# mhnazeri/PMoE

Hardware: AMD Instinct MI355X
Metric: samples/sec fwd+bwd, 256x256 RGB 4-expert PMoE (higher is better)
Workload: dtype bf16; 1 GPU; 4-expert MoE (PMoE experts), 256x256x3 x4 frames, batch 64/GPU, fwd+moe_loss+bwd, dropout 0.3; global_batch=64, parallelism=dp1

## Files before the change

pmoe_amd/csrc/conv_res.hip:

```cpp
#include "conv_common.h"
#include <stdlib.h>
#include "kernels.h"

template <int LOG_RB> __device__ __forceinline__ int rswz(int x) { return swz_chunk<LOG_RB, 0>(x); }

template <int LOG_RB, bool BIAS = false>
__global__ void __launch_bounds__(512) conv3x3_res_kernel(const ConvArgs a, const int tiles_per_expert,
                                                         const int wgs_per_expert, const int region_bytes) {
    constexpr int RB = 1 << LOG_RB, CPR = RB / 16, LOG_CPR = LOG_RB - 4;
    constexpr int KSUB = RB / 32;
    constexpr int VE = 8;
    constexpr int MAXV = 11;
    extern __shared__ __attribute__((aligned(16))) char smem[];

    const int tid = threadIdx.x, lane = tid & 63, wave = tid >> 6;
    const int grp = wave >> 2, gw = wave & 3, gtid = tid & 255;
    const int l31 = lane & 31, hh = lane >> 5;
    const int e = blockIdx.y, wg = blockIdx.x;
    const int t0 = (int)((long long)wg * tiles_per_expert / wgs_per_expert);
    const int t1 = (int)((long long)(wg + 1) * tiles_per_expert / wgs_per_expert);
    const int n = t1 - t0;

    const int lTW = a.lTW, lTH = a.lTH;
    const int TW = 1 << lTW, TH = 1 << lTH;
    const int PW = TW + 2, PH = TH + 2;
    const int NPIX = a.TN * PH * PW;

    char* Wl = smem;
    char* region = smem + 9 * 64 * RB + grp * region_bytes;

    float* lbias = reinterpret_cast<float*>(smem + 9 * 64 * RB + 2 * region_bytes);
    if (BIAS && tid < 64) lbias[tid] = a.bias[(size_t)e * a.CoutP + tid];
    {
        const bf16* wsrc = (const bf16*)a.w + (size_t)e * a.CoutP * 9 * a.Cin;
        for (int v = tid; v < 9 * 64 * CPR; v += 512) {
            const int j = v & (CPR - 1);
            const int row = (v >> LOG_CPR) & 63;
            const int tap = v >> (LOG_CPR + 6);
            const v4i val = ldg16(wsrc + ((size_t)row * 9 + tap) * a.Cin + j * VE);
            *reinterpret_cast<v4i*>(Wl + (tap * 64 + row) * RB + ((j ^ rswz<LOG_RB>(row)) << 4)) = val;
        }
    }

    auto geom = [&](int t, PatchGeom& g, int& n0, int& oy0, int& ox0) {
        int q = t0 + t;
        const int px = q % a.tiles_x; q /= a.tiles_x;
        const int py = q % a.tiles_y; q /= a.tiles_y;
        n0 = e * a.ipe + q * a.TN;
        oy0 = py * TH; ox0 = px * TW;
        g.n0 = n0; g.n_end = (e + 1) * a.ipe; g.e_first_img = e * a.ipe;
        g.Y0 = oy0 - 1; g.X0 = ox0 - 1; g.PH = PH; g.PW = PW; g.NPIX = NPIX;
        g.H = a.H; g.W = a.W; g.ld = a.in_ld; g.coff = a.in_coff; g.cmax = a.Cin;
        g.dilate = 0; g.shared = a.in_shared; g.step = 1;
    };

    const bf16* in = (const bf16*)a.in;
    PatchStage<bf16, LOG_RB, 256, MAXV> ps;
    auto issue_tile = [&](int t) {
        PatchGeom g; int n0, oy0, ox0;
        geom(t, g, n0, oy0, ox0);
        ps.issue(in, g, 0, gtid);
    };

    int ppb[2];
#pragma unroll
    for (int mt = 0; mt < 2; ++mt) {
        const int p = gw * 64 + mt * 32 + l31;
        const int mx = p & (TW - 1), my = (p >> lTW) & (TH - 1), pn = p >> (lTW + lTH);
        ppb[mt] = (pn * PH + my) * PW + mx;
    }
    int arow_off[2][KSUB];
#pragma unroll
    for (int nt = 0; nt < 2; ++nt)
#pragma unroll
        for (int ks = 0; ks < KSUB; ++ks) {
            const int row = nt * 32 + l31;
            arow_off[nt][ks] = row * RB + (((ks * 2 + hh) ^ rswz<LOG_RB>(row)) << 4);
        }

    f32x16 acc[2][2];
    float s1[VE], s2[VE];
#pragma unroll
    for (int i = 0; i < VE; ++i) s1[i] = s2[i] = 0.f;
    const int cc = gtid & 7, pr = gtid >> 3;
    const bool cvalid = cc * VE < a.Cout;
    bf16* out = (bf16*)a.out;
    const bf16* res = (const bf16*)a.res;

    if (grp == 0 && n > 0) {
        issue_tile(0);
        ps.template commit<0>(region, NPIX, gtid);
    }
    __syncthreads();

    auto taps = [&](int tap_lo) {
        int pb[2] = {ppb[0], ppb[1]};
        asm volatile("" : "+v"(pb[0]), "+v"(pb[1]));
#pragma unroll
        for (int tp = 0; tp < 3; ++tp) {
            const int tap = tap_lo + tp;
            const int tapoff = (tap / 3) * PW + (tap % 3);
            const char* wt = Wl + tap * 64 * RB;
            int pp[2], fp[2];
#pragma unroll
            for (int mt = 0; mt < 2; ++mt) {
                pp[mt] = pb[mt] + tapoff;
                fp[mt] = rswz<LOG_RB>(pp[mt]);
            }
#pragma unroll
            for (int ks = 0; ks < KSUB; ++ks) {
                v4i af[2], bfr[2];
#pragma unroll
                for (int nt = 0; nt < 2; ++nt) af[nt] = *reinterpret_cast<const v4i*>(wt + arow_off[nt][ks]);
#pragma unroll
                for (int mt = 0; mt < 2; ++mt)
                    bfr[mt] = *reinterpret_cast<const v4i*>(region + (pp[mt] << LOG_RB) + (((ks * 2 + hh) ^ fp[mt]) << 4));
#pragma unroll
                for (int nt = 0; nt < 2; ++nt)
#pragma unroll
                    for (int mt = 0; mt < 2; ++mt)
                        acc[nt][mt] = __builtin_amdgcn_mfma_f32_32x32x16_bf16(__builtin_bit_cast(bf16x8, af[nt]),
                                                                              __builtin_bit_cast(bf16x8, bfr[mt]),
                                                                              acc[nt][mt], 0, 0, 0);
            }
        }
    };

    for (int h = 0; h <= n; ++h) {
        if (grp == (h & 1)) {
            const bool live = h < n;
            if (live) {
                if (BIAS) {
#pragma unroll
                    for (int i = 0; i < 2; ++i)
#pragma unroll
                        for (int g = 0; g < 4; ++g) {
                            const f32x4 b = *reinterpret_cast<const f32x4*>(lbias + (i * 4 + g) * 8 + hh * 4);
#pragma unroll
                            for (int j = 0; j < 2; ++j)
#pragma unroll
                                for (int k = 0; k < 4; ++k) acc[i][j][4 * g + k] = b[k];
                        }
                } else {
#pragma unroll
                    for (int i = 0; i < 2; ++i)
#pragma unroll
                        for (int j = 0; j < 2; ++j)
#pragma unroll
                            for (int k = 0; k < 16; ++k) acc[i][j][k] = 0.f;
                }
                taps(0);
            }
            __syncthreads();
            if (live) taps(3);
            __syncthreads();
            if (live) taps(6);
            __syncthreads();
        } else {
            const bool have = h >= 1, next = h + 1 < n;
            PatchGeom gg; int n0 = 0, oy0 = 0, ox0 = 0;
            v4i rb[8];
            if (next) issue_tile(h + 1);
            if (have) {
                geom(h - 1, gg, n0, oy0, ox0);
#pragma unroll
                for (int nt = 0; nt < 2; ++nt)
#pragma unroll
                    for (int mt = 0; mt < 2; ++mt) {
                        const int p = gw * 64 + mt * 32 + l31;
#pragma unroll
                        for (int g = 0; g < 4; ++g) {
                            bf16x4 v;
#pragma unroll
                            for (int i = 0; i < 4; ++i) v[i] = (bf16)acc[nt][mt][4 * g + i];
                            *reinterpret_cast<bf16x4*>(region + p * 128 + (((nt * 4 + g) ^ (p & 7)) << 4) + 8 * hh) = v;
                        }
                    }
            }
            __syncthreads();
            if (have) {
#pragma unroll
                for (int u = 0; u < 8; ++u) {
                    const int p = pr + 32 * u;
                    rb[u] = *reinterpret_cast<const v4i*>(region + p * 128 + ((cc ^ (p & 7)) << 4));
                }
            }
            __syncthreads();
            if (next) ps.template commit<0>(region, NPIX, gtid);
            if (have) {
#pragma unroll
                for (int u = 0; u < 8; ++u) {
                    const int p = pr + 32 * u;
                    const int mx = p & (TW - 1), my = (p >> lTW) & (TH - 1), pn = p >> (lTW + lTH);
                    const int nn = n0 + pn, oy = oy0 + my, ox = ox0 + mx;
                    if (cvalid && nn < gg.n_end && oy < a.Ho && ox < a.Wo) {
                        const size_t opix = ((size_t)nn * a.Ho + oy) * a.Wo + ox;
                        v4i pk = rb[u];
                        if (a.res_mode == PMOE_RES_ADD) {
                            float v[VE], rv[VE];
                            unpack16<bf16>(rb[u], v);
                            unpack16<bf16>(ldg16(res + opix * a.res_ld + a.res_coff + cc * VE), rv);
#pragma unroll
                            for (int i = 0; i < VE; ++i) v[i] += rv[i];
                            pk = pack16<bf16>(v);
                        }
                        if (a.stats) {
                            float rr[VE];
                            unpack16<bf16>(pk, rr);
#pragma unroll
                            for (int i = 0; i < VE; ++i) { s1[i] += rr[i]; s2[i] += rr[i] * rr[i]; }
                        }
                        stg16(out + opix * a.out_ld + a.out_coff + cc * VE, pk);
                    }
                }
            }
            __syncthreads();
        }
    }

    if (a.stats) {
        __syncthreads();
        float* red = reinterpret_cast<float*>(smem);
#pragma unroll
        for (int i = 0; i < VE; ++i) {
#pragma unroll
            for (int off = 8; off < 64; off <<= 1) {
                s1[i] += __shfl_xor(s1[i], off);
                s2[i] += __shfl_xor(s2[i], off);
            }
        }
        if (lane < 8) {
#pragma unroll
            for (int i = 0; i < VE; ++i) {
                red[(wave * 2 + 0) * 64 + cc * VE + i] = s1[i];
                red[(wave * 2 + 1) * 64 + cc * VE + i] = s2[i];
            }
        }
        __syncthreads();
        if (tid < 128) {
            const int which = tid >> 6, c = tid & 63;
            float s = 0.f;
#pragma unroll
            for (int w = 0; w < 8; ++w) s += red[(w * 2 + which) * 64 + c];
            a.stats[(((size_t)e * wgs_per_expert + wg) * 2 + which) * a.CoutP + c] = s;
        }
    }
}

#ifdef PMOE_STAMP
#define RSTAMP_INIT unsigned long long st_prev = __builtin_amdgcn_s_memtime(); const unsigned long long st_r0 = __builtin_amdgcn_s_memrealtime(); unsigned st_acc[5] = {0, 0, 0, 0, 0};
#define RLAP(i) { const unsigned long long st_t = __builtin_amdgcn_s_memtime(); st_acc[i] += (unsigned)(st_t - st_prev); st_prev = st_t; }
#else
#define RSTAMP_INIT
#define RLAP(i)
#endif

template <bool BIAS>
__global__ void __launch_bounds__(512, 2) conv3x3_resdma_kernel(const ConvArgs a, const int tiles_per_expert,
                                                                const int wgs_per_expert, const int pbuf_bytes,
                                                                const int magic_pw, const int magic_ph) {
    constexpr int RB = 128, LOG_RBK = 7, VE = 8;
    typedef __attribute__((address_space(3))) void lds_void;
    extern __shared__ __attribute__((aligned(16))) char smem[];
    const int tid = threadIdx.x, lane = tid & 63;
    const int wave = __builtin_amdgcn_readfirstlane(tid >> 6);
    const int l31 = lane & 31, hh = lane >> 5;
    const int wm = wave >> 1, wn = wave & 1;
    const int e = blockIdx.y, wg = blockIdx.x;
    const int t0 = (int)((long long)wg * tiles_per_expert / wgs_per_expert);
    const int t1 = (int)((long long)(wg + 1) * tiles_per_expert / wgs_per_expert);
    const int ntile = t1 - t0;

    const int lTW = a.lTW, lTH = a.lTH;
    const int TW = 1 << lTW, TH = 1 << lTH;
    const int PW = TW + 2, PH = TH + 2;
    const int NPIX = a.TN * PH * PW;
    const int NPIECE = (NPIX + 7) >> 3;
    const int my_pieces = (NPIECE - wave + 7) >> 3;

    char* Wl = smem;
    char* pbuf = smem + 9 * 64 * RB;
    float* lbias = reinterpret_cast<float*>(pbuf + 2 * pbuf_bytes);
    if (BIAS && tid < 64) lbias[tid] = a.bias[(size_t)e * a.CoutP + tid];
    const bool dbn = a.res_mode == PMOE_RES_DBN;
    float* lbn = lbias + 64;
    if (dbn && tid < 256) {
        const int nset = a.N / a.bn_ipe;
        lbn[tid] = (tid & 63) < a.Cout ? a.bn[((size_t)(tid >> 6) * nset + (e * a.ipe) / a.bn_ipe) * a.Cout + (tid & 63)] : 0.f;
    }

    const bf16* inb = (const bf16*)a.in + (size_t)e * a.ipe * a.H * a.W * a.in_ld + a.in_coff;
    const __amdgpu_buffer_rsrc_t rs_in = __builtin_amdgcn_make_buffer_rsrc(
        (void*)inb, (short)0, (int)(((long long)a.ipe * a.H * a.W * a.in_ld - a.in_coff) * 2), 0x00020000);
    const bf16* wsrc = (const bf16*)a.w + (size_t)e * a.CoutP * 9 * a.Cin;
    const __amdgpu_buffer_rsrc_t rs_w = __builtin_amdgcn_make_buffer_rsrc((void*)wsrc, (short)0, 64 * 9 * 64 * 2, 0x00020000);
    constexpr int OOB = 0x7ff80000;

#pragma unroll
    for (int i = 0; i < 9; ++i) {
        const int piece = wave + 8 * i;
        const int tap = piece >> 3, row = ((piece & 7) << 3) + (lane >> 3);
        const int voff = ((row * 9 + tap) * 64 * 2) + (((lane & 7) ^ ((row >> 1) & 7)) << 4);
        __builtin_amdgcn_raw_ptr_buffer_load_lds(rs_w, (lds_void*)(Wl + (piece << 10)), 16, voff, 0, 0, 0);
    }

    auto tile_geo = [&](int t, int& n0, int& oy0, int& ox0) {
        int qq = t0 + t;
        const int px = qq % a.tiles_x; qq /= a.tiles_x;
        const int py = qq % a.tiles_y; qq /= a.tiles_y;
        n0 = qq * a.TN;
        oy0 = py * TH; ox0 = px * TW;
    };
    auto issue_patch = [&](int t, int buf) {
        int n0, oy0, ox0;
        tile_geo(t, n0, oy0, ox0);
#pragma unroll
        for (int i = 0; i < 6; ++i) {
            if (i < my_pieces) {
                const int pp = ((wave + 8 * i) << 3) + (lane >> 3);
                const int rowq = (pp * magic_pw) >> 16, px = pp - rowq * PW;
                const int pn = (rowq * magic_ph) >> 16, prow = rowq - pn * PH;
                const int n = n0 + pn, Y = oy0 - 1 + prow, X = ox0 - 1 + px;
                const bool ok = pp < NPIX && n < a.ipe && (unsigned)Y < (unsigned)a.H && (unsigned)X < (unsigned)a.W;
                const int voff = ok ? ((((n * a.H + Y) * a.W + X) * a.in_ld) << 1) + (((lane & 7) ^ ((px >> 1) & 7)) << 4) : OOB;
                __builtin_amdgcn_raw_ptr_buffer_load_lds(rs_in, (lds_void*)(pbuf + buf * pbuf_bytes + ((wave + 8 * i) << 10)), 16,
                                                         voff, 0, 0, 0);
            }
        }
    };

    int pbase[2], pcol[2];
#pragma unroll
    for (int mt = 0; mt < 2; ++mt) {
        const int p = wm * 64 + mt * 32 + l31;
        const int mx = p & (TW - 1), my = (p >> lTW) & (TH - 1), pn = p >> (lTW + lTH);
        pbase[mt] = ((pn * PH + my) * PW + mx) << LOG_RBK;
        pcol[mt] = mx;
    }
    int aoff[4];
#pragma unroll
    for (int ks = 0; ks < 4; ++ks) {
        const int row = wn * 32 + l31;
        aoff[ks] = row * RB + (((ks * 2 + hh) ^ ((row >> 1) & 7)) << 4);
    }

    float s1[VE], s2[VE];
#pragma unroll
    for (int i = 0; i < VE; ++i) s1[i] = s2[i] = 0.f;
    const int cc = tid & 7, pr = tid >> 3;
    const bool cvalid = cc * VE < a.Cout;
    bf16* out = (bf16*)a.out;
    const bf16* res = (const bf16*)a.res;
    const bool res_pref = (a.res_mode == PMOE_RES_ADD || dbn) && a.prefetch;

    if (ntile > 0) issue_patch(0, 0);
    asm volatile("s_waitcnt vmcnt(0) lgkmcnt(0)" ::: "memory");
    __builtin_amdgcn_s_barrier();
    float kmu[VE], kis[VE], ksc[VE], ksh[VE];
#pragma unroll
    for (int i = 0; i < VE; ++i) kmu[i] = kis[i] = ksc[i] = ksh[i] = 0.f;
    if (dbn) {
#pragma unroll
        for (int i = 0; i < VE; ++i) {
            kmu[i] = lbn[cc * VE + i]; kis[i] = lbn[64 + cc * VE + i]; ksc[i] = lbn[128 + cc * VE + i]; ksh[i] = lbn[192 + cc * VE + i];
        }
    }

    RSTAMP_INIT
    for (int t = 0; t < ntile; ++t) {
        const int buf = t & 1;
        if (t + 1 < ntile) issue_patch(t + 1, buf ^ 1);
        v4i rpre[4];
        if (res_pref) {
            int n0, oy0, ox0;
            tile_geo(t, n0, oy0, ox0);
#pragma unroll
            for (int u = 0; u < 4; ++u) {
                const int p = pr + 64 * u;
                const int mx = p & (TW - 1), my = (p >> lTW) & (TH - 1), pn = p >> (lTW + lTH);
                const int nn = n0 + pn, oy = oy0 + my, ox = ox0 + mx;
                rpre[u] = v4i{0, 0, 0, 0};
                if (cvalid && nn < a.ipe && oy < a.Ho && ox < a.Wo)
                    rpre[u] = ldg16(res + ((((size_t)e * a.ipe + nn) * a.Ho + oy) * a.Wo + ox) * a.res_ld + a.res_coff + cc * VE);
            }
        }
        const char* patch = pbuf + buf * pbuf_bytes;
        f32x16 acc[2];
        if (BIAS) {
#pragma unroll
            for (int g = 0; g < 4; ++g) {
                const f32x4 b = *reinterpret_cast<const f32x4*>(lbias + wn * 32 + g * 8 + hh * 4);
#pragma unroll
                for (int mt = 0; mt < 2; ++mt)
#pragma unroll
                    for (int k = 0; k < 4; ++k) acc[mt][4 * g + k] = b[k];
            }
        } else {
#pragma unroll
            for (int mt = 0; mt < 2; ++mt)
#pragma unroll
                for (int k = 0; k < 16; ++k) acc[mt][k] = 0.f;
        }
        RLAP(0)
        auto read_step = [&](int st, v4i& af, v4i* bfr) {
            const int tap = st >> 2, ks = st & 3;
            const int tapoff = ((tap / 3) * PW + (tap % 3)) << LOG_RBK;
            af = *reinterpret_cast<const v4i*>(Wl + tap * 64 * RB + aoff[ks]);
#pragma unroll
            for (int mt = 0; mt < 2; ++mt)
                bfr[mt] = *reinterpret_cast<const v4i*>(patch + pbase[mt] + tapoff +
                                                        (((ks * 2 + hh) ^ (((pcol[mt] + (tap % 3)) >> 1) & 7)) << 4));
        };
#pragma unroll
        for (int st = 0; st < 36; ++st) {
            v4i af, bfr[2];
            read_step(st, af, bfr);
#pragma unroll
            for (int mt = 0; mt < 2; ++mt)
                acc[mt] = __builtin_amdgcn_mfma_f32_32x32x16_bf16(__builtin_bit_cast(bf16x8, af), __builtin_bit_cast(bf16x8, bfr[mt]),
                                                                  acc[mt], 0, 0, 0);
        }
        char* stage = pbuf + buf * pbuf_bytes;
        RLAP(1)
        asm volatile("s_waitcnt lgkmcnt(0)" ::: "memory");
        __builtin_amdgcn_s_barrier();
        RLAP(2)
#pragma unroll
        for (int mt = 0; mt < 2; ++mt) {
            const int p = wm * 64 + mt * 32 + l31;
#pragma unroll
            for (int g = 0; g < 4; ++g) {
                bf16x4 v;
#pragma unroll
                for (int i = 0; i < 4; ++i) v[i] = (bf16)acc[mt][4 * g + i];
                *reinterpret_cast<bf16x4*>(stage + p * 128 + (((wn * 4 + g) ^ (p & 7)) << 4) + 8 * hh) = v;
            }
        }
        asm volatile("s_waitcnt vmcnt(0) lgkmcnt(0)" ::: "memory");
        __builtin_amdgcn_s_barrier();
        RLAP(3)
        int n0, oy0, ox0;
        tile_geo(t, n0, oy0, ox0);
#pragma unroll
        for (int u = 0; u < 4; ++u) {
            const int p = pr + 64 * u;
            const v4i raw = *reinterpret_cast<const v4i*>(stage + p * 128 + ((cc ^ (p & 7)) << 4));
            const int mx = p & (TW - 1), my = (p >> lTW) & (TH - 1), pn = p >> (lTW + lTH);
            const int nn = n0 + pn, oy = oy0 + my, ox = ox0 + mx;
            if (cvalid && nn < a.ipe && oy < a.Ho && ox < a.Wo) {
                const size_t opix = (((size_t)e * a.ipe + nn) * a.Ho + oy) * a.Wo + ox;
                v4i pk = raw;
                if (dbn) {
                    float v[VE], rv[VE];
                    unpack16<bf16>(raw, v);
                    unpack16<bf16>(res_pref ? rpre[u] : ldg16(res + opix * a.res_ld + a.res_coff + cc * VE), rv);
#pragma unroll
                    for (int i = 0; i < VE; ++i) {
                        const float d = rv[i] - kmu[i];
                        const float gq = (d * ksc[i] + ksh[i]) > 0.f ? v[i] : 0.f;
                        v[i] = gq;
                        s1[i] += gq;
                        s2[i] += gq * (d * kis[i]);
                    }
                    pk = pack16<bf16>(v);
                } else {
                if (a.res_mode == PMOE_RES_ADD) {
                    float v[VE], rv[VE];
                    unpack16<bf16>(raw, v);
                    unpack16<bf16>(res_pref ? rpre[u] : ldg16(res + opix * a.res_ld + a.res_coff + cc * VE), rv);
#pragma unroll
                    for (int i = 0; i < VE; ++i) v[i] += rv[i];
                    pk = pack16<bf16>(v);
                }
                if (a.stats) {
                    float rr[VE];
                    unpack16<bf16>(pk, rr);
#pragma unroll
                    for (int i = 0; i < VE; ++i) { s1[i] += rr[i]; s2[i] += rr[i] * rr[i]; }
                }
                }
                stg16(out + opix * a.out_ld + a.out_coff + cc * VE, pk);
            }
        }
        asm volatile("s_waitcnt lgkmcnt(0)" ::: "memory");
        __builtin_amdgcn_s_barrier();
        RLAP(4)
    }
#ifdef PMOE_STAMP
    if (a.stats && lane == 0) {
        float* o = a.stats + (((size_t)e * wgs_per_expert + wg) * 8 + wave) * 8;
        for (int i = 0; i < 5; ++i) o[i] = (float)st_acc[i];
        o[5] = (float)(unsigned)(__builtin_amdgcn_s_memrealtime() - st_r0);
        o[6] = (float)ntile;
    }
    return;
#endif

    if (a.stats) {
        __syncthreads();
        float* red = reinterpret_cast<float*>(smem);
#pragma unroll
        for (int i = 0; i < VE; ++i) {
#pragma unroll
            for (int off = 8; off < 64; off <<= 1) {
                s1[i] += __shfl_xor(s1[i], off);
                s2[i] += __shfl_xor(s2[i], off);
            }
        }
        if (lane < 8) {
#pragma unroll
            for (int i = 0; i < VE; ++i) {
                red[(wave * 2 + 0) * 64 + cc * VE + i] = s1[i];
                red[(wave * 2 + 1) * 64 + cc * VE + i] = s2[i];
            }
        }
        __syncthreads();
        if (tid < 128) {
            const int which = tid >> 6, c = tid & 63;
            float s = 0.f;
#pragma unroll
            for (int w = 0; w < 8; ++w) s += red[(w * 2 + which) * 64 + c];
            a.stats[(((size_t)e * wgs_per_expert + wg) * 2 + which) * a.CoutP + c] = s;
        }
    }
}

template <bool BIAS, int MODE, bool RZ_LATE = true>
__global__ void __launch_bounds__(512, 2) conv3x3_respipe_kernel(const ConvArgs a, const int tiles_per_expert,
                                                                 const int wgs_per_expert, const int pbuf_bytes,
                                                                 const int magic_pw, const int magic_ph) {
    constexpr int RB = 128, LOG_RBK = 7;
    typedef __attribute__((address_space(3))) void lds_void;
    typedef unsigned v4u __attribute__((ext_vector_type(4)));
    typedef float f32x2 __attribute__((ext_vector_type(2)));
    extern __shared__ __attribute__((aligned(16))) char smem[];
    const int tid = threadIdx.x, lane = tid & 63;
    const int wave = __builtin_amdgcn_readfirstlane(tid >> 6);
    const int l31 = lane & 31, hh = lane >> 5;
    const int wm = wave >> 1, wn = wave & 1;
    const int e = blockIdx.y, wg = blockIdx.x;
    const int t0 = (int)((long long)wg * tiles_per_expert / wgs_per_expert);
    const int t1 = (int)((long long)(wg + 1) * tiles_per_expert / wgs_per_expert);
    const int ntile = t1 - t0;

    const int lTW = a.lTW, lTH = a.lTH;
    const int TW = 1 << lTW, TH = 1 << lTH;
    const int PW = TW + 2, PH = TH + 2;
    const int NPIX = a.TN * PH * PW;
    const int NPIECE = (NPIX + 7) >> 3;
    const int my_pieces = (NPIECE - wave + 7) >> 3;

    char* Wl = smem;
    char* pbuf = smem + 9 * 64 * RB;
    float* lbias = reinterpret_cast<float*>(pbuf + 2 * pbuf_bytes);
    if (BIAS && tid < 64) lbias[tid] = a.bias[(size_t)e * a.CoutP + tid];
    float* lbn = lbias + 64;
    if (MODE == 2 && tid < 256) {
        const int nset = a.N / a.bn_ipe;
        lbn[tid] = (tid & 63) < a.Cout ? a.bn[((size_t)(tid >> 6) * nset + (e * a.ipe) / a.bn_ipe) * a.Cout + (tid & 63)] : 0.f;
    }
    constexpr bool HASRES = MODE == 1 || MODE == 2, INBN = MODE == 3;
    if (INBN && tid < 256) {
        const int nset = a.N / a.bn_ipe;
        lbn[tid] = a.bn[((size_t)(tid >> 6) * nset + (e * a.ipe) / a.bn_ipe) * a.Cin + (tid & 63)];
    }

    constexpr int OOB = 0x7ff80000;
    const bf16* inb = (const bf16*)a.in + (size_t)e * a.ipe * a.H * a.W * a.in_ld + a.in_coff;
    const __amdgpu_buffer_rsrc_t rs_in = __builtin_amdgcn_make_buffer_rsrc(
        (void*)inb, (short)0, (int)(((long long)a.ipe * a.H * a.W * a.in_ld - a.in_coff) * 2), 0x00020000);
    const bf16* wsrc = (const bf16*)a.w + (size_t)e * a.CoutP * 9 * a.Cin;
    const __amdgpu_buffer_rsrc_t rs_w = __builtin_amdgcn_make_buffer_rsrc((void*)wsrc, (short)0, 64 * 9 * 64 * 2, 0x00020000);
    bf16* outb = (bf16*)a.out + (size_t)e * a.ipe * a.Ho * a.Wo * a.out_ld + a.out_coff;
    const __amdgpu_buffer_rsrc_t rs_out = __builtin_amdgcn_make_buffer_rsrc(
        (void*)outb, (short)0, (int)(((long long)a.ipe * a.Ho * a.Wo * a.out_ld - a.out_coff) * 2), 0x00020000);
    const bf16* resb = HASRES ? (const bf16*)a.res + (size_t)e * a.ipe * a.Ho * a.Wo * a.res_ld + a.res_coff : (const bf16*)a.in;
    const __amdgpu_buffer_rsrc_t rs_res = __builtin_amdgcn_make_buffer_rsrc(
        (void*)resb, (short)0, HASRES ? (int)(((long long)a.ipe * a.Ho * a.Wo * a.res_ld - a.res_coff) * 2) : 0, 0x00020000);

#pragma unroll
    for (int i = 0; i < 9; ++i) {
        const int piece = wave + 8 * i;
        const int tap = piece >> 3, row = ((piece & 7) << 3) + (lane >> 3);
        const int voff = ((row * 9 + tap) * 64 * 2) + (((lane & 7) ^ ((row >> 1) & 7)) << 4);
        __builtin_amdgcn_raw_ptr_buffer_load_lds(rs_w, (lds_void*)(Wl + (piece << 10)), 16, voff, 0, 0, 0);
    }

    int prel[6], pgeo[6];
#pragma unroll
    for (int i = 0; i < 6; ++i) {
        const int pp = ((wave + 8 * i) << 3) + (lane >> 3);
        const int rowq = (pp * magic_pw) >> 16, px = pp - rowq * PW;
        const int pn = (rowq * magic_ph) >> 16, prow = rowq - pn * PH;
        prel[i] = ((((pn * a.H + prow) * a.W + px) * a.in_ld) << 1) + (((lane & 7) ^ ((px >> 1) & 7)) << 4);
        pgeo[i] = pp < NPIX ? (pn << 20) | (prow << 10) | px : (0x7ff << 20);
    }
    struct Walk { int px, py, q; };
    Walk cur;
    {
        int qq = t0;
        cur.px = qq % a.tiles_x; qq /= a.tiles_x;
        cur.py = qq % a.tiles_y; cur.q = qq / a.tiles_y;
    }
    auto advance = [&](Walk w) {
        if (++w.px == a.tiles_x) { w.px = 0; if (++w.py == a.tiles_y) { w.py = 0; ++w.q; } }
        return w;
    };
    auto issue_patch = [&](const Walk& w, int buf) {
        const int n0 = w.q * a.TN, Y0 = w.py * TH - 1, X0 = w.px * TW - 1;
        const int tbase = (((n0 * a.H + Y0) * a.W + X0) * a.in_ld) << 1;
#pragma unroll
        for (int i = 0; i < 6; ++i) {
            if (i < my_pieces) {
                const int n = n0 + (pgeo[i] >> 20), Y = Y0 + ((pgeo[i] >> 10) & 0x3ff), X = X0 + (pgeo[i] & 0x3ff);
                const bool ok = n < a.ipe && (unsigned)Y < (unsigned)a.H && (unsigned)X < (unsigned)a.W;
                __builtin_amdgcn_raw_ptr_buffer_load_lds(rs_in, (lds_void*)(pbuf + buf * pbuf_bytes + ((wave + 8 * i) << 10)), 16,
                                                         ok ? tbase + prel[i] : OOB, 0, 0, 0);
            }
        }
    };

    int pbase[2], pcol[2];
    unsigned ovo[2], rvo[2];
    int ogeo[2];
#pragma unroll
    for (int mt = 0; mt < 2; ++mt) {
        const int p = wm * 64 + mt * 32 + l31;
        const int mx = p & (TW - 1), my = (p >> lTW) & (TH - 1), pn = p >> (lTW + lTH);
        pbase[mt] = ((pn * PH + my) * PW + mx) << LOG_RBK;
        pcol[mt] = mx;
        const int orel = (pn * a.Ho + my) * a.Wo + mx;
        ogeo[mt] = (pn << 20) | (my << 10) | mx;
        ovo[mt] = (unsigned)(orel * a.out_ld + wn * 32 + 8 * hh) * 2u;
        rvo[mt] = (unsigned)(orel * a.res_ld + wn * 32 + 8 * hh) * 2u;
    }
    const int c0 = wn * 32 + 8 * hh;
    const bool cval[2] = {c0 < a.Cout, c0 + 16 < a.Cout};
    int aoff[4];
#pragma unroll
    for (int ks = 0; ks < 4; ++ks) {
        const int row = wn * 32 + l31;
        aoff[ks] = row * RB + (((ks * 2 + hh) ^ ((row >> 1) & 7)) << 4);
    }

    f32x2 s1[2][4], s2[2][4];
#pragma unroll
    for (int k = 0; k < 2; ++k)
#pragma unroll
        for (int q = 0; q < 4; ++q) s1[k][q] = s2[k][q] = f32x2{0.f, 0.f};

    auto unpack2 = [](unsigned w) { return f32x2{__builtin_bit_cast(float, w << 16), __builtin_bit_cast(float, w & 0xffff0000u)}; };
    auto pack2 = [](f32x2 v) {
        typedef __bf16 bf16x2 __attribute__((ext_vector_type(2)));
        return __builtin_bit_cast(unsigned, bf16x2{(bf16)v[0], (bf16)v[1]});
    };
    f32x2 cmu[4], csc[4], csh[4];
    auto xform_coef = [&]() {
#pragma unroll
        for (int q = 0; q < 4; ++q) {
            cmu[q] = *reinterpret_cast<const f32x2*>(lbn + (lane & 7) * 8 + 2 * q);
            csc[q] = *reinterpret_cast<const f32x2*>(lbn + 128 + (lane & 7) * 8 + 2 * q);
            csh[q] = *reinterpret_cast<const f32x2*>(lbn + 192 + (lane & 7) * 8 + 2 * q);
        }
    };
    auto xform_addr = [&](int buf, const int i) {
        const int ii = i < 5 || i < my_pieces ? i : 0;
        const int px = (i < 5 || i < my_pieces ? pgeo[i] : pgeo[0]) & 0x3ff;
        return pbuf + buf * pbuf_bytes + ((wave + 8 * ii) << 10) + ((lane >> 3) << 7) + (((lane & 7) ^ ((px >> 1) & 7)) << 4);
    };
    auto xform_load = [&](int buf, const int i) { return *reinterpret_cast<const v4u*>(xform_addr(buf, i)); };
    auto xform_store = [&](const Walk& w, int buf, const int i, const v4u z) {
        const int n0 = w.q * a.TN, Y0 = w.py * TH - 1, X0 = w.px * TW - 1;
        const int n = n0 + (pgeo[i] >> 20), Y = Y0 + ((pgeo[i] >> 10) & 0x3ff), X = X0 + (pgeo[i] & 0x3ff);
        const bool ok = n < a.ipe && (unsigned)Y < (unsigned)a.H && (unsigned)X < (unsigned)a.W;
        typedef short s16x2 __attribute__((ext_vector_type(2)));
        v4u o;
#pragma unroll
        for (int q = 0; q < 4; ++q) {
            const f32x2 v = __builtin_elementwise_fma(unpack2(z[q]) - cmu[q], csc[q], csh[q]);
            const unsigned pk = __builtin_bit_cast(unsigned, __builtin_elementwise_max(__builtin_bit_cast(s16x2, pack2(v)), s16x2{0, 0}));
            o[q] = i < 5 || i < my_pieces ? pk : z[q];
        }
        if (ok || !(i < 5 || i < my_pieces)) *reinterpret_cast<v4u*>(xform_addr(buf, i)) = o;
    };

    if (ntile > 0) issue_patch(cur, 0);
    asm volatile("s_waitcnt vmcnt(0) lgkmcnt(0)" ::: "memory");
    if (INBN && ntile > 0) {
        __builtin_amdgcn_s_barrier();
        xform_coef();
#pragma unroll
        for (int i = 0; i < 6; ++i) xform_store(cur, 0, i, xform_load(0, i));
        asm volatile("s_waitcnt lgkmcnt(0)" ::: "memory");
    }
    __builtin_amdgcn_s_barrier();

    v4u prev[2][2], rprev[2][2];
    bool pval[2] = {false, false};
    unsigned psoff = 0;
#pragma unroll
    for (int mt = 0; mt < 2; ++mt)
#pragma unroll
        for (int k = 0; k < 2; ++k) prev[mt][k] = rprev[mt][k] = v4u{0u, 0u, 0u, 0u};

    auto readout = [&](const int k) {
        v4u pk[2];
        const bool ok[2] = {pval[0] && cval[k], pval[1] && cval[k]};
#pragma unroll
        for (int q = 0; q < 4; ++q) {
            f32x2 mu, is, sc, sh;
            if (MODE == 2) {
                mu = *reinterpret_cast<const f32x2*>(lbn + c0 + 16 * k + 2 * q);
                is = *reinterpret_cast<const f32x2*>(lbn + 64 + c0 + 16 * k + 2 * q);
                sc = *reinterpret_cast<const f32x2*>(lbn + 128 + c0 + 16 * k + 2 * q);
                sh = *reinterpret_cast<const f32x2*>(lbn + 192 + c0 + 16 * k + 2 * q);
            }
#pragma unroll
            for (int mt = 0; mt < 2; ++mt) {
                const unsigned w = ok[mt] ? prev[mt][k][q] : 0u;
                f32x2 v = unpack2(w);
                if (MODE == 2) {
                    const f32x2 d = unpack2(rprev[mt][k][q]) - mu;
                    const f32x2 y = __builtin_elementwise_fma(d, sc, sh);
                    v = f32x2{y[0] > 0.f ? v[0] : 0.f, y[1] > 0.f ? v[1] : 0.f};
                    s1[k][q] += v;
                    s2[k][q] = __builtin_elementwise_fma(v, d * is, s2[k][q]);
                    pk[mt][q] = pack2(v);
                } else if (MODE == 1) {
                    v += unpack2(rprev[mt][k][q]);
                    pk[mt][q] = pack2(v);
                } else {
                    pk[mt][q] = w;
                    s1[k][q] += v;
                    s2[k][q] = __builtin_elementwise_fma(v, v, s2[k][q]);
                }
            }
        }
#pragma unroll
        for (int mt = 0; mt < 2; ++mt)
            __builtin_amdgcn_raw_buffer_store_b128(pk[mt], rs_out, (int)(ok[mt] ? ovo[mt] + psoff + 32u * k : (unsigned)OOB), 0, 0);
    };

    RSTAMP_INIT
    for (int t = 0; t < ntile; ++t) {
        const int buf = t & 1;
        const Walk nxt = advance(cur);
        if (t + 1 < ntile) issue_patch(nxt, buf ^ 1);
        const int n0 = cur.q * a.TN, oy0 = cur.py * TH, ox0 = cur.px * TW;
        const unsigned osoff = (unsigned)(((n0 * a.Ho + oy0) * a.Wo + ox0) * a.out_ld) * 2u;
        bool val[2];
        v4u rz[2][2];
#pragma unroll
        for (int mt = 0; mt < 2; ++mt) {
            val[mt] = n0 + (ogeo[mt] >> 20) < a.ipe && oy0 + ((ogeo[mt] >> 10) & 0x3ff) < a.Ho && ox0 + (ogeo[mt] & 0x3ff) < a.Wo;
        }
        const unsigned rsoff = HASRES ? (unsigned)(((n0 * a.Ho + oy0) * a.Wo + ox0) * a.res_ld) * 2u : 0u;
        auto load_rz = [&](const int mt) {
#pragma unroll
            for (int k = 0; k < 2; ++k)
                rz[mt][k] = __builtin_amdgcn_raw_buffer_load_b128(rs_res, (int)(val[mt] && cval[k] ? rvo[mt] : (unsigned)OOB),
                                                                  (int)(rsoff + 32u * k), 0);
        };
        if (HASRES && !RZ_LATE) { load_rz(0); load_rz(1); }
        const char* patch = pbuf + buf * pbuf_bytes;
        f32x16 acc[2];
        if (BIAS) {
#pragma unroll
            for (int g = 0; g < 4; ++g) {
                const f32x4 b = *reinterpret_cast<const f32x4*>(lbias + wn * 32 + g * 8 + hh * 4);
#pragma unroll
                for (int mt = 0; mt < 2; ++mt)
#pragma unroll
                    for (int k = 0; k < 4; ++k) acc[mt][4 * g + k] = b[k];
            }
        } else {
#pragma unroll
            for (int mt = 0; mt < 2; ++mt)
#pragma unroll
                for (int k = 0; k < 16; ++k) acc[mt][k] = 0.f;
        }
        RLAP(0)
        v4u xz = v4u{0u, 0u, 0u, 0u};
#pragma unroll
        for (int st = 0; st < 36; ++st) {
            const int tap = st >> 2, ks = st & 3;
            const int tapoff = ((tap / 3) * PW + (tap % 3)) << LOG_RBK;
            const v4i af = *reinterpret_cast<const v4i*>(Wl + tap * 64 * RB + aoff[ks]);
            v4i bfr[2];
#pragma unroll
            for (int mt = 0; mt < 2; ++mt)
                bfr[mt] = *reinterpret_cast<const v4i*>(patch + pbase[mt] + tapoff +
                                                        (((ks * 2 + hh) ^ (((pcol[mt] + (tap % 3)) >> 1) & 7)) << 4));
#pragma unroll
            for (int mt = 0; mt < 2; ++mt)
                acc[mt] = __builtin_amdgcn_mfma_f32_32x32x16_bf16(__builtin_bit_cast(bf16x8, af), __builtin_bit_cast(bf16x8, bfr[mt]),
                                                                  acc[mt], 0, 0, 0);
            if (st == 3) readout(0);
            if (st == 11) readout(1);
            if (st == 19) __builtin_amdgcn_sched_barrier(0);
            if (HASRES && RZ_LATE && st == 22) load_rz(0);
            if (HASRES && RZ_LATE && st == 26) load_rz(1);
            if (INBN && t + 1 < ntile) {
                if (st == 19) { asm volatile("s_waitcnt vmcnt(4)" ::: "memory"); xform_coef(); }
                if (st >= 20 && st < 32) {
                    if (!(st & 1)) xz = xform_load(buf ^ 1, (st - 20) >> 1);
                    else xform_store(nxt, buf ^ 1, (st - 20) >> 1, xz);
                }
            }
        }
        RLAP(1)
#pragma unroll
        for (int mt = 0; mt < 2; ++mt) {
#pragma unroll
            for (int k = 0; k < 2; ++k) {
                unsigned x[2], y[2];
#pragma unroll
                for (int d = 0; d < 2; ++d) {
                    x[d] = pack2(f32x2{acc[mt][8 * k + 2 * d], acc[mt][8 * k + 2 * d + 1]});
                    y[d] = pack2(f32x2{acc[mt][8 * k + 4 + 2 * d], acc[mt][8 * k + 4 + 2 * d + 1]});
                    const auto r = __builtin_amdgcn_permlane32_swap(x[d], y[d], false, false);
                    x[d] = r[0]; y[d] = r[1];
                }
                prev[mt][k] = v4u{x[0], x[1], y[0], y[1]};
                if (HASRES) rprev[mt][k] = rz[mt][k];
            }
            pval[mt] = val[mt];
        }
        psoff = osoff;
        cur = nxt;
        if (HASRES && RZ_LATE) asm volatile("s_waitcnt vmcnt(4) lgkmcnt(0)" ::: "memory");
        else
        asm volatile("s_waitcnt vmcnt(0) lgkmcnt(0)" ::: "memory");
        __builtin_amdgcn_s_barrier();
        RLAP(2)
    }
    readout(0);
    readout(1);
#ifdef PMOE_STAMP
    if (a.stats && lane == 0) {
        float* o = a.stats + (((size_t)e * wgs_per_expert + wg) * 8 + wave) * 8;
        for (int i = 0; i < 5; ++i) o[i] = (float)st_acc[i];
        o[5] = (float)(unsigned)(__builtin_amdgcn_s_memrealtime() - st_r0);
        o[6] = (float)ntile;
    }
    return;
#endif

    if (a.stats) {
        __syncthreads();
        float* red = reinterpret_cast<float*>(smem);
#pragma unroll
        for (int k = 0; k < 2; ++k)
#pragma unroll
            for (int q = 0; q < 4; ++q)
#pragma unroll
                for (int c = 0; c < 2; ++c) {
                    float u = s1[k][q][c], v = s2[k][q][c];
#pragma unroll
                    for (int off = 1; off < 32; off <<= 1) {
                        u += __shfl_xor(u, off);
                        v += __shfl_xor(v, off);
                    }
                    if (l31 == 0) {
                        red[(wave * 2 + 0) * 64 + c0 + 16 * k + 2 * q + c] = u;
                        red[(wave * 2 + 1) * 64 + c0 + 16 * k + 2 * q + c] = v;
                    }
                }
        __syncthreads();
        if (tid < 128) {
            const int which = tid >> 6, c = tid & 63;
            float s = 0.f;
#pragma unroll
            for (int w = 0; w < 4; ++w) s += red[((w * 2 + (c >> 5)) * 2 + which) * 64 + c];
            a.stats[(((size_t)e * wgs_per_expert + wg) * 2 + which) * a.CoutP + c] = s;
        }
    }
}

bool conv_res_plan(const ConvArgs& a, int dtype, ConvLaunch* l) {
    if (dtype != PMOE_DT_BF16 || a.ks != 3 || a.stride != 1 || a.pad != 1 || a.dilate) return false;
    if (a.CoutP != 64 || a.Cout % 8 || (a.Cin != 64 && a.Cin != 16)) return false;
    if (a.act != PMOE_ACT_NONE || a.drop_p > 0.f) return false;
    if (a.bias && ((a.res_mode != PMOE_RES_NONE && a.res_mode != PMOE_RES_DBN) || a.Cin != 64)) return false;
    if (a.res_mode != PMOE_RES_NONE && a.res_mode != PMOE_RES_ADD && a.res_mode != PMOE_RES_DBN && a.res_mode != PMOE_RES_INBN) return false;
    if (a.res_mode == PMOE_RES_DBN && a.Cin != 64) return false;
    if (a.res_mode == PMOE_RES_INBN && (a.Cin != 64 || a.in_shared || !a.bn)) return false;
    if (a.N % a.ipe || a.Ho != a.H || a.Wo != a.W) return false;
    const PixelTile t = pixel_tile(a.Ho, a.Wo, a.ipe, 8, 5);
    const int PW = patch_extent(t.lTW, 3, 1), PH = patch_extent(t.lTH, 3, 1);
    const int NPIX = t.TN * PH * PW;
    const int log_rb = a.Cin == 64 ? 7 : 5;
    const int rb = 1 << log_rb, cpr = rb / 16;
    if (NPIX * cpr > 11 * 256) return false;
    size_t region = (size_t)NPIX * rb;
    if (region < 256 * 128) region = 256 * 128;
    region = (region + 255) & ~(size_t)255;
    const size_t smem = (size_t)9 * 64 * rb + 2 * region;
    if (smem + (a.bias ? 256 : 0) > 163840) return false;
    const int E = a.N / a.ipe;
    ResPlan& p = l->res;
    p.tiles_per_expert = t.per_expert();
    int wpe = 256 / E; if (wpe < 1) wpe = 1;
    if (wpe > p.tiles_per_expert) wpe = p.tiles_per_expert;
    p.wgs_per_expert = wpe;
    p.log_rb = log_rb;
    p.smem = smem;
    ConvArgs& c = l->a;
    c = a;
    set_tile(c, t);
    l->kind = CONV_RES;
    l->mblocks = E * wpe;

    const int npiece = (NPIX + 7) / 8;
    int pb = npiece * 1024;
    if (pb < 256 * 128) pb = 256 * 128;
    const size_t sm = (size_t)9 * 64 * 128 + 2 * (size_t)pb + 256 + 1024;
    l->res_dma = p.log_rb == 7 && !a.in_shared && sw("PMOE_RES_DMA", 1) && magic_div_exact(npiece * 8, PW, PH, &l->mpw, &l->mph) &&
                 npiece <= 48 && sm <= 163840 && t.lTW >= 4 && (long long)a.ipe * a.H * a.W * a.in_ld * 2 < 0x7ff00000ll;
    if (l->res_dma) { l->pbuf = pb; l->smem = sm; }
    l->res_pipe = l->res_dma && sw("PMOE_RES_PIPE", 1) && a.ipe <= 2047 && !(a.res_mode == PMOE_RES_ADD && a.stats) &&
                  (long long)a.ipe * a.Ho * a.Wo * a.out_ld * 2 < 0x7ff00000ll &&
                  (a.res_mode == PMOE_RES_NONE || (long long)a.ipe * a.Ho * a.Wo * a.res_ld * 2 < 0x7ff00000ll);
    if (l->res_dma && !l->res_pipe) c.prefetch = 1;
    const int mode = a.res_mode == PMOE_RES_INBN ? 3 : a.res_mode == PMOE_RES_DBN ? 2 : a.res_mode == PMOE_RES_ADD ? 1 : 0;
    l->code = 1000 + p.log_rb + (l->res_dma ? (l->res_pipe ? 200 + 20 * mode : 100) + (a.bias ? 10 : 0) : 0);
    return true;
}

template <bool BIAS, int MODE> static int launch_respipe(const ConvLaunch& l, dim3 grid, hipStream_t st) {
    return launch<conv3x3_respipe_kernel<BIAS, MODE>>(grid, dim3(512), l.smem, st, l.a, l.res.tiles_per_expert, l.res.wgs_per_expert,
                                                       l.pbuf, l.mpw, l.mph);
}

int conv_res_launch(const ConvLaunch& l, hipStream_t st) {
    const ConvArgs& a = l.a;
    const ResPlan& p = l.res;
    const int E = a.N / a.ipe;
    dim3 grid(p.wgs_per_expert, E), block(512);
    if (l.res_pipe) {
        const int mode = a.res_mode == PMOE_RES_DBN ? 2 : a.res_mode == PMOE_RES_ADD ? 1 : 0;
        if (a.res_mode == PMOE_RES_INBN) return launch_respipe<false, 3>(l, grid, st);
        if (a.bias) return mode == 2 ? launch_respipe<true, 2>(l, grid, st)
                         : mode == 1 ? launch_respipe<true, 1>(l, grid, st)
                                     : launch_respipe<true, 0>(l, grid, st);
        return mode == 2 ? launch_respipe<false, 2>(l, grid, st)
             : mode == 1 ? launch_respipe<false, 1>(l, grid, st)
                         : launch_respipe<false, 0>(l, grid, st);
    }
    if (l.res_dma) {
        if (a.bias) return launch<conv3x3_resdma_kernel<true>>(grid, block, l.smem, st, a, p.tiles_per_expert, p.wgs_per_expert, l.pbuf, l.mpw, l.mph);
        return launch<conv3x3_resdma_kernel<false>>(grid, block, l.smem, st, a, p.tiles_per_expert, p.wgs_per_expert, l.pbuf, l.mpw, l.mph);
    }
    const int region = (int)((p.smem - (size_t)9 * 64 * (1 << p.log_rb)) / 2);
    if (p.log_rb == 7 && a.bias)
        return launch<conv3x3_res_kernel<7, true>>(grid, block, p.smem + 256, st, a, p.tiles_per_expert, p.wgs_per_expert, region);
    if (p.log_rb == 7) return launch<conv3x3_res_kernel<7, false>>(grid, block, p.smem, st, a, p.tiles_per_expert, p.wgs_per_expert, region);
    return launch<conv3x3_res_kernel<5, false>>(grid, block, p.smem, st, a, p.tiles_per_expert, p.wgs_per_expert, region);
}
```

Baseline: 1914 samples/s.

## Add producer waves issuing patch DMA in residual conv pipeline kernel

For residual modes 1 and 2, the conv3x3 respipe kernel gets four extra producer waves (768 threads) that only issue the buffer-to-LDS patch loads for the next tile, then meet the eight MFMA consumer waves at a barrier. The consumers stop issuing patch loads and no longer wait on vmcnt for them, so their load latency is hidden behind compute. Mode 2 also precomputes the swizzled LDS B and A offsets per dx, replacing per-step index math with XOR on ks. Residual loads now land directly in rprev. The cost is higher launch bounds and register pressure, plus tighter barrier coupling between the two wave roles.

```diff
diff --git a/pmoe_amd/csrc/conv_res.hip b/pmoe_amd/csrc/conv_res.hip
--- a/pmoe_amd/csrc/conv_res.hip
+++ b/pmoe_amd/csrc/conv_res.hip
@@ -1,5 +1,6 @@
 #include "conv_common.h"
 #include <stdlib.h>
+#include <type_traits>
 #include "kernels.h"
 
 template <int LOG_RB> __device__ __forceinline__ int rswz(int x) { return swz_chunk<LOG_RB, 0>(x); }
@@ -250,6 +251,14 @@
 #ifdef PMOE_STAMP
 #define RSTAMP_INIT unsigned long long st_prev = __builtin_amdgcn_s_memtime(); const unsigned long long st_r0 = __builtin_amdgcn_s_memrealtime(); unsigned st_acc[5] = {0, 0, 0, 0, 0};
 #define RLAP(i) { const unsigned long long st_t = __builtin_amdgcn_s_memtime(); st_acc[i] += (unsigned)(st_t - st_prev); st_prev = st_t; }
+#define RSTAMP_OUT(role)                                                                                     \
+    if (a.stats && lane == 0) {                                                                              \
+        float* o = a.stats + (((size_t)e * wgs_per_expert + wg) * 16 + wave) * 8;                            \
+        for (int i = 0; i < 5; ++i) o[i] = (float)st_acc[i];                                                 \
+        o[5] = (float)(unsigned)(__builtin_amdgcn_s_memrealtime() - st_r0);                                  \
+        o[6] = (float)ntile;                                                                                 \
+        o[7] = (float)(role);                                                                                \
+    }
 #else
 #define RSTAMP_INIT
 #define RLAP(i)
@@ -525,10 +534,12 @@
     }
 }
 
-template <bool BIAS, int MODE, bool RZ_LATE = true>
-__global__ void __launch_bounds__(512, 2) conv3x3_respipe_kernel(const ConvArgs a, const int tiles_per_expert,
-                                                                 const int wgs_per_expert, const int pbuf_bytes,
-                                                                 const int magic_pw, const int magic_ph) {
+constexpr int RESPIPE_REQ_WAVES = 4;
+template <bool BIAS, int MODE, bool PROD = false>
+__global__ void __launch_bounds__(PROD ? 512 + 64 * RESPIPE_REQ_WAVES : 512, PROD ? 3 : 2)
+conv3x3_respipe_kernel(const ConvArgs a, const int tiles_per_expert, const int wgs_per_expert, const int pbuf_bytes,
+                       const int magic_pw, const int magic_ph) {
+    static_assert(!(PROD && MODE == 3), "mode 3 transforms the pieces its own wave requested: 8-wave form only");
     constexpr int RB = 128, LOG_RBK = 7;
     typedef __attribute__((address_space(3))) void lds_void;
     typedef unsigned v4u __attribute__((ext_vector_type(4)));
@@ -578,6 +589,75 @@
     const __amdgpu_buffer_rsrc_t rs_res = __builtin_amdgcn_make_buffer_rsrc(
         (void*)resb, (short)0, HASRES ? (int)(((long long)a.ipe * a.Ho * a.Wo * a.res_ld - a.res_coff) * 2) : 0, 0x00020000);
 
+    struct Walk { int px, py, q; };
+    auto walk_start = [&]() {
+        Walk w;
+        int qq = t0;
+        w.px = qq % a.tiles_x; qq /= a.tiles_x;
+        w.py = qq % a.tiles_y; w.q = qq / a.tiles_y;
+        return w;
+    };
+    auto advance = [&](Walk w) {
+        if (++w.px == a.tiles_x) { w.px = 0; if (++w.py == a.tiles_y) { w.py = 0; ++w.q; } }
+        return w;
+    };
+    auto piece_geometry = [&](auto npc, int* prel, int* pgeo, const int w0, const int stride) {
+#pragma unroll
+        for (int i = 0; i < decltype(npc)::value; ++i) {
+            const int pp = ((w0 + stride * i) << 3) + (lane >> 3);
+            const int rowq = (pp * magic_pw) >> 16, px = pp - rowq * PW;
+            const int pn = (rowq * magic_ph) >> 16, prow = rowq - pn * PH;
+            prel[i] = ((((pn * a.H + prow) * a.W + px) * a.in_ld) << 1) + (((lane & 7) ^ ((px >> 1) & 7)) << 4);
+            pgeo[i] = pp < NPIX ? (pn << 20) | (prow << 10) | px : (0x7ff << 20);
+        }
+    };
+    auto issue_pieces = [&](auto npc, const int* prel, const int* pgeo, const int w0, const int stride, const int cnt, const Walk& w,
+                            const int buf) {
+        const int n0 = w.q * a.TN, Y0 = w.py * TH - 1, X0 = w.px * TW - 1;
+        const int tbase = (((n0 * a.H + Y0) * a.W + X0) * a.in_ld) << 1;
+#pragma unroll
+        for (int i = 0; i < decltype(npc)::value; ++i) {
+            if (i < cnt) {
+                const int n = n0 + (pgeo[i] >> 20), Y = Y0 + ((pgeo[i] >> 10) & 0x3ff), X = X0 + (pgeo[i] & 0x3ff);
+                const bool ok = n < a.ipe && (unsigned)Y < (unsigned)a.H && (unsigned)X < (unsigned)a.W;
+                __builtin_amdgcn_raw_ptr_buffer_load_lds(rs_in, (lds_void*)(pbuf + buf * pbuf_bytes + ((w0 + stride * i) << 10)), 16,
+                                                         ok ? tbase + prel[i] : OOB, 0, 0, 0);
+            }
+        }
+    };
+
+    if (PROD && wave >= 8) {
+        constexpr int NQ = 48 / RESPIPE_REQ_WAVES;
+        const std::integral_constant<int, NQ> np;
+        const int r = wave - 8, cnt = (NPIECE - r + RESPIPE_REQ_WAVES - 1) / RESPIPE_REQ_WAVES;
+        int qrel[NQ], qgeo[NQ];
+        piece_geometry(np, qrel, qgeo, r, RESPIPE_REQ_WAVES);
+        Walk cur = walk_start();
+        __builtin_amdgcn_s_setprio(2);
+        if (ntile > 0) issue_pieces(np, qrel, qgeo, r, RESPIPE_REQ_WAVES, cnt, cur, 0);
+        asm volatile("s_waitcnt vmcnt(0)" ::: "memory");
+        __builtin_amdgcn_s_barrier();
+        RSTAMP_INIT
+        for (int t = 0; t < ntile; ++t) {
+            cur = advance(cur);
+            if (t + 1 < ntile) issue_pieces(np, qrel, qgeo, r, RESPIPE_REQ_WAVES, cnt, cur, (t & 1) ^ 1);
+            RLAP(0)
+            asm volatile("s_waitcnt vmcnt(0)" ::: "memory");
+            RLAP(1)
+            __builtin_amdgcn_s_barrier();
+            RLAP(2)
+        }
+#ifdef PMOE_STAMP
+        RSTAMP_OUT(1)
+        return;
+#endif
+        if (a.stats) {
+            __builtin_amdgcn_s_barrier();
+            __builtin_amdgcn_s_barrier();
+        }
+        return;
+    }
+
 #pragma unroll
     for (int i = 0; i < 9; ++i) {
         const int piece = wave + 8 * i;
@@ -595,17 +675,12 @@
         prel[i] = ((((pn * a.H + prow) * a.W + px) * a.in_ld) << 1) + (((lane & 7) ^ ((px >> 1) & 7)) << 4);
         pgeo[i] = pp < NPIX ? (pn << 20) | (prow << 10) | px : (0x7ff << 20);
     }
-    struct Walk { int px, py, q; };
     Walk cur;
     {
         int qq = t0;
         cur.px = qq % a.tiles_x; qq /= a.tiles_x;
         cur.py = qq % a.tiles_y; cur.q = qq / a.tiles_y;
     }
-    auto advance = [&](Walk w) {
-        if (++w.px == a.tiles_x) { w.px = 0; if (++w.py == a.tiles_y) { w.py = 0; ++w.q; } }
-        return w;
-    };
     auto issue_patch = [&](const Walk& w, int buf) {
         const int n0 = w.q * a.TN, Y0 = w.py * TH - 1, X0 = w.px * TW - 1;
         const int tbase = (((n0 * a.H + Y0) * a.W + X0) * a.in_ld) << 1;
@@ -642,6 +717,12 @@
         const int row = wn * 32 + l31;
         aoff[ks] = row * RB + (((ks * 2 + hh) ^ ((row >> 1) & 7)) << 4);
     }
+    constexpr bool LEAN = PROD && MODE == 2;
+    int bx[3][2];
+#pragma unroll
+    for (int dx = 0; dx < 3; ++dx)
+#pragma unroll
+        for (int mt = 0; mt < 2; ++mt) bx[dx][mt] = pbase[mt] + ((hh ^ (((pcol[mt] + dx) >> 1) & 7)) << 4);
 
     f32x2 s1[2][4], s2[2][4];
 #pragma unroll
@@ -684,7 +765,7 @@
         if (ok || !(i < 5 || i < my_pieces)) *reinterpret_cast<v4u*>(xform_addr(buf, i)) = o;
     };
 
-    if (ntile > 0) issue_patch(cur, 0);
+    if (!PROD && ntile > 0) issue_patch(cur, 0);
     asm volatile("s_waitcnt vmcnt(0) lgkmcnt(0)" ::: "memory");
     if (INBN && ntile > 0) {
         __builtin_amdgcn_s_barrier();
@@ -745,7 +826,7 @@
     for (int t = 0; t < ntile; ++t) {
         const int buf = t & 1;
         const Walk nxt = advance(cur);
-        if (t + 1 < ntile) issue_patch(nxt, buf ^ 1);
+        if (!PROD && t + 1 < ntile) issue_patch(nxt, buf ^ 1);
         const int n0 = cur.q * a.TN, oy0 = cur.py * TH, ox0 = cur.px * TW;
         const unsigned osoff = (unsigned)(((n0 * a.Ho + oy0) * a.Wo + ox0) * a.out_ld) * 2u;
         bool val[2];
@@ -758,10 +839,9 @@
         auto load_rz = [&](const int mt) {
 #pragma unroll
             for (int k = 0; k < 2; ++k)
-                rz[mt][k] = __builtin_amdgcn_raw_buffer_load_b128(rs_res, (int)(val[mt] && cval[k] ? rvo[mt] : (unsigned)OOB),
+                (PROD ? rprev : rz)[mt][k] = __builtin_amdgcn_raw_buffer_load_b128(rs_res, (int)(val[mt] && cval[k] ? rvo[mt] : (unsigned)OOB),
                                                                   (int)(rsoff + 32u * k), 0);
         };
-        if (HASRES && !RZ_LATE) { load_rz(0); load_rz(1); }
         const char* patch = pbuf + buf * pbuf_bytes;
         f32x16 acc[2];
         if (BIAS) {
@@ -785,12 +865,15 @@
         for (int st = 0; st < 36; ++st) {
             const int tap = st >> 2, ks = st & 3;
             const int tapoff = ((tap / 3) * PW + (tap % 3)) << LOG_RBK;
-            const v4i af = *reinterpret_cast<const v4i*>(Wl + tap * 64 * RB + aoff[ks]);
+            if (LEAN && st % 12 == 0)
+                asm volatile("" : "+v"(bx[0][0]), "+v"(bx[0][1]), "+v"(bx[1][0]), "+v"(bx[1][1]), "+v"(bx[2][0]), "+v"(bx[2][1]), "+v"(aoff[0]));
+            const v4i af = *reinterpret_cast<const v4i*>(Wl + tap * 64 * RB + (LEAN ? aoff[0] ^ (ks << 5) : aoff[ks]));
             v4i bfr[2];
 #pragma unroll
             for (int mt = 0; mt < 2; ++mt)
-                bfr[mt] = *reinterpret_cast<const v4i*>(patch + pbase[mt] + tapoff +
-                                                        (((ks * 2 + hh) ^ (((pcol[mt] + (tap % 3)) >> 1) & 7)) << 4));
+                bfr[mt] = LEAN ? *reinterpret_cast<const v4i*>(patch + tapoff + (bx[tap % 3][mt] ^ (ks << 5)))
+                               : *reinterpret_cast<const v4i*>(patch + pbase[mt] + tapoff +
+                                                               (((ks * 2 + hh) ^ (((pcol[mt] + (tap % 3)) >> 1) & 7)) << 4));
 #pragma unroll
             for (int mt = 0; mt < 2; ++mt)
                 acc[mt] = __builtin_amdgcn_mfma_f32_32x32x16_bf16(__builtin_bit_cast(bf16x8, af), __builtin_bit_cast(bf16x8, bfr[mt]),
@@ -798,8 +881,8 @@
             if (st == 3) readout(0);
             if (st == 11) readout(1);
             if (st == 19) __builtin_amdgcn_sched_barrier(0);
-            if (HASRES && RZ_LATE && st == 22) load_rz(0);
-            if (HASRES && RZ_LATE && st == 26) load_rz(1);
+            if (HASRES && st == 22) load_rz(0);
+            if (HASRES && st == 26) load_rz(1);
             if (INBN && t + 1 < ntile) {
                 if (st == 19) { asm volatile("s_waitcnt vmcnt(4)" ::: "memory"); xform_coef(); }
                 if (st >= 20 && st < 32) {
@@ -822,27 +905,22 @@
                     x[d] = r[0]; y[d] = r[1];
                 }
                 prev[mt][k] = v4u{x[0], x[1], y[0], y[1]};
-                if (HASRES) rprev[mt][k] = rz[mt][k];
+                if (HASRES && !PROD) rprev[mt][k] = rz[mt][k];
             }
             pval[mt] = val[mt];
         }
         psoff = osoff;
         cur = nxt;
-        if (HASRES && RZ_LATE) asm volatile("s_waitcnt vmcnt(4) lgkmcnt(0)" ::: "memory");
-        else
-        asm volatile("s_waitcnt vmcnt(0) lgkmcnt(0)" ::: "memory");
+        if (PROD) asm volatile("s_waitcnt lgkmcnt(0)" ::: "memory");
+        else if (HASRES) asm volatile("s_waitcnt vmcnt(4) lgkmcnt(0)" ::: "memory");
+        else asm volatile("s_waitcnt vmcnt(0) lgkmcnt(0)" ::: "memory");
         __builtin_amdgcn_s_barrier();
         RLAP(2)
     }
     readout(0);
     readout(1);
 #ifdef PMOE_STAMP
-    if (a.stats && lane == 0) {
-        float* o = a.stats + (((size_t)e * wgs_per_expert + wg) * 8 + wave) * 8;
-        for (int i = 0; i < 5; ++i) o[i] = (float)st_acc[i];
-        o[5] = (float)(unsigned)(__builtin_amdgcn_s_memrealtime() - st_r0);
-        o[6] = (float)ntile;
-    }
+    RSTAMP_OUT(0)
     return;
 #endif
 
@@ -927,9 +1005,12 @@
     return true;
 }
 
+constexpr bool respipe_prod(bool bias, int mode) { return mode == 1 || mode == 2; }
+
 template <bool BIAS, int MODE> static int launch_respipe(const ConvLaunch& l, dim3 grid, hipStream_t st) {
-    return launch<conv3x3_respipe_kernel<BIAS, MODE>>(grid, dim3(512), l.smem, st, l.a, l.res.tiles_per_expert, l.res.wgs_per_expert,
-                                                       l.pbuf, l.mpw, l.mph);
+    constexpr bool PROD = respipe_prod(BIAS, MODE);
+    return launch<conv3x3_respipe_kernel<BIAS, MODE, PROD>>(grid, dim3(PROD ? 512 + 64 * RESPIPE_REQ_WAVES : 512), l.smem, st, l.a, l.res.tiles_per_expert,
+                                                             l.res.wgs_per_expert, l.pbuf, l.mpw, l.mph);
 }
 
 int conv_res_launch(const ConvLaunch& l, hipStream_t st) {
```

After: 1930 samples/s, median of 5. No clear change (+0.8%).
